# ThorsteinnJonsson/SLAM_framework

Hardware: AMD Instinct MI355X
Metric: stereo frames/sec ORB extract+match @1241x376, 2000 kp/frame (higher is better)
Workload: dtype u8; 1 GPU; configs[1]: synthetic 1241x376 stereo stream, 2000 kp/frame, extract L+R + stereo match + frame-to-frame match; batch=256, streams=1, batches_in_flight=2, nfeatures=2000, nlevels=8, parallelism=frame-sharded x1

## Files before the change

### slam_framework_amd/csrc/orb_kernels.hip

```cpp
#include <hip/hip_runtime.h>
#include <stdint.h>

#include <type_traits>
#include <utility>
#include <cstdlib>

#include "device_math.h"
#include "timing.h"
#include "orb_geometry.h"
#include "orb_kernels.h"

namespace slamgpu {

__constant__ __attribute__((aligned(16))) int8_t c_pattern[1024] = {
#include "orb_pattern.inc"
};

__device__ __forceinline__ const uint8_t* level_ptr(const ImageBatch& b, const OrbGeom* g,
                                                    int img, int level, int* pitch) {
  if (level == 0) {
    *pitch = b.in_pitch;
    return batch_image(b, img);
  }
  *pitch = g->lv[level].pitch;
// ... 992 lines not shown
      const int U = block_scan_array<kThr>(S.b, m, S.wsum);
      const int E = block_scan_array<kThr>(S.c, m, S.wsum);
      const int newm = T + U;
      const int seq0 = S.seq_next;
      const bool ovf = newm > min(2 * L.node_cap, kOctCap) || E > kOctCap;
      if (!ovf) {
        for (int j = tid; j < m; j += kThr) {
          const OctNode nd = Lc[j];
          if (nd.n > 1) {
            int gpos = S.a[j], epos = S.c[j];
            for (int q = 0; q < 4; q++) {
              OctNode ch = child[4 * j + q];
              if (ch.n == 0) continue;
              ch.seq = seq0 + gpos;
              const int pos = T - 1 - gpos;
              Ln[pos] = ch;
              if (ch.n > 1) S.sortk[epos++] = (uint64_t)pos;
              gpos++;
            }
          } else {
            Ln[T + S.b[j]] = nd;
          }
        }
      }
      __syncthreads();
      if (tid == 0) {
        if (ovf) {
          atomicOr(err, kErrNodeOverflow);
          S.finish = 1;
        } else {
          S.m = newm;
          S.seq_next = seq0 + T;
          S.nexp = E;
          if (newm >= N || newm == m) S.finish = 1;
          else if (newm + E * 3 > N) S.mode = 1;
        }
      }
      if (!ovf) cur ^= 1;
      __syncthreads();
      if (S.finish) break;
    } else {
      const int V = S.nexp;
      int P2 = 1;
      while (P2 < V) P2 <<= 1;
      for (int i = tid; i < P2; i += kThr) {
        uint64_t key = 0;
        if (i < V) {
          const int pos = (int)S.sortk[i];
          const OctNode& nd = Lc[pos];
          key = ((uint64_t)nd.n << 44) | ((uint64_t)(uint32_t)nd.seq << 12) | (uint64_t)pos;
        }
        S.sortk[i] = key;
      }
      __syncthreads();
      for (int k = 2; k <= P2; k <<= 1) {
        for (int jj = k >> 1; jj > 0; jj >>= 1) {
          for (int i = tid; i < P2; i += kThr) {
            const int ixj = i ^ jj;
            if (ixj > i) {
              const uint64_t x = S.sortk[i], y = S.sortk[ixj];
              const bool desc = (i & k) == 0;
              if (desc ? (x < y) : (x > y)) {
                S.sortk[i] = y;
                S.sortk[ixj] = x;
              }
            }
          }
          __syncthreads();
        }
      }
      for (int j = wid; j < V; j += (kThr / 64)) {
        const int pos = (int)(S.sortk[j] & 0xfff);
        const OctNode nd = Lc[pos];
        OctNode ch[4];
        divide_wave(nd, keys, ch, lane);
        if (lane == 0) {
          int t = 0, e = 0;
          for (int q = 0; q < 4; q++) {
            child[4 * j + q] = ch[q];
            t += ch[q].n > 0;
            e += ch[q].n > 1;
          }
          S.a[j] = t;
          S.c[j] = e;
          S.b[j] = t - 1;
        }
      }
      __syncthreads();
      for (int i = tid; i < V; i += kThr) S.b[i] = S.a[i] - 1;
      __syncthreads();
      block_scan_array<kThr>(S.b, V, S.wsum);
      if (tid == 0) S.total = V - 1;
      __syncthreads();
      for (int j = tid; j < V; j += kThr)
        if (m + S.b[j] + (S.a[j] - 1) >= N) atomicMin(&S.total, j);
      __syncthreads();
      const int J = S.total;
      const int nproc = J + 1;
      for (int i = tid; i < V; i += kThr)
        if (i >= nproc) {
          S.a[i] = 0;
          S.c[i] = 0;
        }
      __syncthreads();
      const int T = block_scan_array<kThr>(S.a, V, S.wsum);
      const int E = block_scan_array<kThr>(S.c, V, S.wsum);
      for (int i = tid; i < m; i += kThr) S.b[i] = 1;
      __syncthreads();
      for (int j = tid; j < nproc; j += kThr) S.b[(int)(S.sortk[j] & 0xfff)] = 0;
      __syncthreads();
      const int U = block_scan_array<kThr>(S.b, m, S.wsum);
      const int newm = T + U;
      const int seq0 = S.seq_next;
      const bool ovf = newm > min(2 * L.node_cap, kOctCap) || E > kOctCap;
      __shared__ uint8_t processed[kOctCap];
      for (int i = tid; i < m; i += kThr) processed[i] = 0;
      __syncthreads();
      for (int j = tid; j < nproc; j += kThr) processed[(int)(S.sortk[j] & 0xfff)] = 1;
      __syncthreads();
      __shared__ int vnext[kOctCap];
      if (!ovf) {
        for (int j = tid; j < nproc; j += kThr) {
          int gpos = S.a[j], epos = S.c[j];
          for (int q = 0; q < 4; q++) {
            OctNode ch = child[4 * j + q];
            if (ch.n == 0) continue;
            ch.seq = seq0 + gpos;
            const int pos = T - 1 - gpos;
            Ln[pos] = ch;
            if (ch.n > 1) vnext[epos++] = pos;
            gpos++;
          }
        }
        for (int i = tid; i < m; i += kThr)
          if (!processed[i]) Ln[T + S.b[i]] = Lc[i];
      }
      __syncthreads();
      for (int i = tid; i < E; i += kThr) S.sortk[i] = (uint64_t)vnext[i];
      __syncthreads();
      if (tid == 0) {
        if (ovf) {
          atomicOr(err, kErrNodeOverflow);
          S.finish = 1;
        } else {
          S.m = newm;
          S.seq_next = seq0 + T;
          S.nexp = E;
          if (newm >= N || newm == m) S.finish = 1;
        }
      }
      if (!ovf) cur ^= 1;
      __syncthreads();
      if (S.finish) break;
    }
  }
  const int m = S.m;
  const OctNode* Lf = lists[cur];
  const int mout = min(m, L.out_cap);
  for (int j = tid; j < mout; j += kThr) {
    const OctNode nd = Lf[j];
    const uint32_t* ks = keys[nd.buf] + nd.kbeg;
    uint32_t best = ks[0];
    for (int k = 1; k < nd.n; k++) {
      const uint32_t kk = ks[k];
      if (key_score(kk) > key_score(best)) best = kk;
    }
    outk[j] = best;
  }
  if (tid == 0) {
    if (m > L.out_cap) atomicOr(err, kErrNodeOverflow);
    *outc = mout;
  }
}

constexpr int kOctFbMaxGroups = 256;
__global__ __launch_bounds__(kOctThreads) void octree_kernel(
    const OrbGeom* __restrict__ g, int n_images, const uint32_t* __restrict__ cell_keys,
    const int* __restrict__ cell_count, uint32_t* __restrict__ key_scratch,
    OctNode* __restrict__ node_scratch, uint32_t* __restrict__ oct_keys,
    int* __restrict__ oct_count, uint32_t* __restrict__ err) {
  __shared__ OctShared S;
  __shared__ int s_todo[kOctThreads];
  __shared__ int s_wcnt[kOctWaves];
  const int tid = threadIdx.x, wid = tid >> 6, lane = tid & 63, nlev = g->nlevels;
  const int total = n_images * nlev;
  const int G = gridDim.x;
  for (int j0 = 0; (int)blockIdx.x + j0 * G < total; j0 += kOctThreads) {
    const int e = (int)blockIdx.x + (j0 + tid) * G;
    const bool redo = e < total && oct_count[e] == -1;
    const uint64_t m = __ballot(redo);
    if (lane == 0) s_wcnt[wid] = __popcll(m);
    __syncthreads();
    int off = 0, nt = 0;
    for (int w = 0; w < kOctWaves; w++) {
      if (w < wid) off += s_wcnt[w];
      nt += s_wcnt[w];
    }
    if (redo) s_todo[off + lanes_below(m)] = e;
    __syncthreads();
    for (int i = 0; i < nt; i++) {
      const int ei = s_todo[i];
      octree_global<kOctThreads>(S, ei % nlev, ei / nlev, g, cell_keys, cell_count, key_scratch,
                                 node_scratch, oct_keys, oct_count, err);
      __syncthreads();
    }
    __syncthreads();
  }
}

#ifndef OCT_PROF
#define OCT_PROF 0
#endif
#ifndef OCT_LANE_KEYS
#define OCT_LANE_KEYS 64
#endif
constexpr int kOctLaneKeys = OCT_LANE_KEYS;
constexpr int kOctDivRegs = 16;

struct OctNodeS {
  int16_t x0, x1, y0, y1;
  uint32_t kn;
};
static_assert(sizeof(OctNodeS) == 12, "compact node");
__device__ __forceinline__ int node_kbeg(const OctNodeS& d) { return (int)(d.kn & 0xffffu); }
__device__ __forceinline__ int node_n(const OctNodeS& d) { return (int)(d.kn >> 16); }

__device__ __forceinline__ OctNodeS readlane_node(const OctNodeS& nd, int l) {
  uint32_t w[3];
  __builtin_memcpy(w, &nd, sizeof(w));
#pragma unroll
  for (int i = 0; i < 3; i++) w[i] = (uint32_t)__builtin_amdgcn_readlane((int)w[i], l);
  OctNodeS o;
  __builtin_memcpy(&o, w, sizeof(w));
  return o;
}

__device__ __forceinline__ int quadrant(uint32_t k, int xm, int ym) {
  return (key_x(k) >= xm ? 1 : 0) + (key_y(k) >= ym ? 2 : 0);
}
__device__ __forceinline__ int node_xm(const OctNodeS& d) { return d.x0 + ((d.x1 - d.x0 + 1) >> 1); }
__device__ __forceinline__ int node_ym(const OctNodeS& d) { return d.y0 + ((d.y1 - d.y0 + 1) >> 1); }

__device__ __forceinline__ int wave_excl_scan(int v, int lane, int* total) {
  int x = v;
  x += __builtin_amdgcn_update_dpp(0, x, 0x111, 0xf, 0xf, false);
  x += __builtin_amdgcn_update_dpp(0, x, 0x112, 0xf, 0xf, false);
  x += __builtin_amdgcn_update_dpp(0, x, 0x114, 0xf, 0xf, false);
  x += __builtin_amdgcn_update_dpp(0, x, 0x118, 0xf, 0xf, false);
  x += __builtin_amdgcn_update_dpp(0, x, 0x142, 0xa, 0xf, false);
  x += __builtin_amdgcn_update_dpp(0, x, 0x143, 0xc, 0xf, false);
  *total = __builtin_amdgcn_readlane(x, 63);
  (void)lane;
  return x - v;
}

__device__ __forceinline__ int wave_scan_array(int16_t* a, int n, int lane) {
  int carry = 0;
  for (int c = 0; c < n; c += 64) {
    const int i = c + lane;
    const int v = i < n ? a[i] : 0;
    int tot;
    const int ex = wave_excl_scan(v, lane, &tot);
    if (i < n) a[i] = (int16_t)(carry + ex);
    carry += tot;
  }
  return carry;
}

__device__ __forceinline__ uint32_t lane_divide(const OctNodeS& nd, uint32_t* keys, bool part) {
  const int xm = node_xm(nd), ym = node_ym(nd), kb = node_kbeg(nd), n = node_n(nd);
  uint32_t kr[kOctLaneKeys];
  uint32_t c = 0;
#pragma unroll
  for (int r = 0; r < kOctLaneKeys; r++)
    if (r < n) {
      kr[r] = keys[kb + r];
      c += 1u << (8 * quadrant(kr[r], xm, ym));
    }
  if (part) {
    uint32_t run = (c << 8) + (c << 16) + (c << 24);
#pragma unroll
    for (int r = 0; r < kOctLaneKeys; r++)
      if (r < n) {
        const int q = quadrant(kr[r], xm, ym);
        keys[kb + ((run >> (8 * q)) & 255)] = kr[r];
        run += 1u << (8 * q);
      }
  }
  return c;
}

__device__ __forceinline__ void wave_count(const OctNodeS& nd, const uint32_t* keys, int lane,
                                           int cnt[4]) {
  const int xm = node_xm(nd), ym = node_ym(nd), kb = node_kbeg(nd), n = node_n(nd);
#pragma unroll
  for (int q = 0; q < 4; q++) cnt[q] = 0;
  for (int s0 = 0; s0 < n; s0 += 64) {
    const int q = s0 + lane < n ? quadrant(keys[kb + s0 + lane], xm, ym) : -1;
#pragma unroll
    for (int qq = 0; qq < 4; qq++) cnt[qq] += __popcll(__ballot(q == qq));
  }
}

__device__ void wave_partition(const OctNodeS& nd, uint32_t* keys, uint32_t* gscratch, int lane,
                               int cnt[4]) {
  const int xm = node_xm(nd), ym = node_ym(nd), kb = node_kbeg(nd), n = node_n(nd);
  if (n <= 64 * kOctDivRegs) {
    const int R = (n + 63) >> 6;
    uint32_t kr[kOctDivRegs];
    int qr[kOctDivRegs];
#pragma unroll
    for (int r = 0; r < kOctDivRegs; r++) {
      qr[r] = -1;
      if (r < R && 64 * r + lane < n) {
        kr[r] = keys[kb + 64 * r + lane];
        qr[r] = quadrant(kr[r], xm, ym);
      }
    }
#pragma unroll
    for (int q = 0; q < 4; q++) cnt[q] = 0;
#pragma unroll
    for (int r = 0; r < kOctDivRegs; r++)
      if (r < R) {
#pragma unroll
        for (int q = 0; q < 4; q++) cnt[q] += __popcll(__ballot(qr[r] == q));
      }
    int run[4] = {0, cnt[0], cnt[0] + cnt[1], cnt[0] + cnt[1] + cnt[2]};
#pragma unroll
    for (int r = 0; r < kOctDivRegs; r++)
      if (r < R) {
#pragma unroll
        for (int q = 0; q < 4; q++) {
          const uint64_t m = __ballot(qr[r] == q);
          if (qr[r] == q) keys[kb + run[q] + lanes_below(m)] = kr[r];
          run[q] += __popcll(m);
        }
      }
  } else {
    wave_count(nd, keys, lane, cnt);
    int run[4] = {0, cnt[0], cnt[0] + cnt[1], cnt[0] + cnt[1] + cnt[2]};
    for (int i = lane; i < n; i += 64) gscratch[kb + i] = keys[kb + i];
    __builtin_amdgcn_fence(__ATOMIC_SEQ_CST, "agent");
    for (int s0 = 0; s0 < n; s0 += 64) {
      const int i = s0 + lane;
      uint32_t k = 0;
      int q = -1;
      if (i < n) {
        k = gscratch[kb + i];
        q = quadrant(k, xm, ym);
      }
#pragma unroll
      for (int qq = 0; qq < 4; qq++) {
        const uint64_t m = __ballot(q == qq);
        if (q == qq) keys[kb + run[qq] + lanes_below(m)] = k;
        run[qq] += __popcll(m);
      }
    }
  }
}

__global__ __launch_bounds__(64 * kMaxLevels) void octree_img_kernel(
    const OrbGeom* __restrict__ g, const uint32_t* __restrict__ cell_keys,
    const int* __restrict__ cell_count, uint32_t* __restrict__ key_scratch,
    uint32_t* __restrict__ oct_keys, int* __restrict__ oct_count, uint32_t* __restrict__ err) {
  extern __shared__ __attribute__((aligned(16))) uint8_t s_oct[];
  __shared__ int s_K[kMaxLevels];
  const int img = blockIdx.x, lane = threadIdx.x & 63, level = wave_id();
  const int nlev = g->nlevels;
  const bool active = level < nlev;
  const LevelGeom& L = g->lv[active ? level : 0];
  const int ncell = L.ncols * L.nrows;
  const int64_t cbase = (int64_t)img * g->cells_per_image + L.cell_base;
#if OCT_PROF
  uint64_t op_t = clock64(), op_acc[8] = {0, 0, 0, 0, 0, 0, 0, 0};
  int op_np = 0, op_V = 0;
  uint32_t op_pass[8][6] = {};
  auto optick = [&](int i) {
    const uint64_t t = clock64();
    op_acc[i] += t - op_t;
    if (i >= 2 && i <= 5 && op_np >= 1 && op_np <= 8) op_pass[op_np - 1][i] += (uint32_t)(t - op_t);
    op_t = t;
  };
#else
  auto optick = [](int) {};
#endif
  int K = 0;
  if (active) {
    for (int c = lane; c < ncell; c += 64) K += cell_count[cbase + c];
    K = wave_sum(K);
    if (lane == 0) s_K[level] = K;
  }
  __syncthreads();
  if (!active) return;
  optick(0);
  int* const outc = oct_count + img * nlev + level;
  uint32_t* const outk = oct_keys + (int64_t)img * g->out_per_image + L.out_base;
  const int nIni = L.n_ini;
  int koff = 0;
  bool fits = true;
  for (int l = 0; l <= level; l++) {
    const bool f = koff + s_K[l] <= g->oct_kcap;
    if (l == level) fits = f;
    else if (f) koff += s_K[l];
  }
  if (!fits || nIni > 16) {
    if (lane == 0) *outc = -1;
    return;
  }
  if (K == 0) {
    if (lane == 0) *outc = 0;
    return;
  }
  uint32_t* const keys = reinterpret_cast<uint32_t*>(s_oct) + koff;
  uint32_t* const gscratch = key_scratch + img * g->keys_per_image + L.key_base;
  const int NC = L.oct_nc;
  OctNodeS* const lists = reinterpret_cast<OctNodeS*>(s_oct + L.oct_list_off);
  uint32_t* const sortk = reinterpret_cast<uint32_t*>(s_oct + L.oct_work_off);
  int16_t* const pt = reinterpret_cast<int16_t*>(sortk + NC);
  int16_t* const pe = pt + NC;
  int16_t* const pu = pe + NC;
  int16_t* const vnext = pu + NC;
  uint8_t* const processed = reinterpret_cast<uint8_t*>(vnext + NC);

  const float hX = L.hx;
  constexpr int kGatherChunks = 8, kGatherRegs = 48;
  constexpr int kMaxGroups = 64 * kGatherChunks / kCellGroup;
  static_assert(kMaxGroups >= 2 && (kMaxGroups & (kMaxGroups - 1)) == 0,
                "the gather's binary search halves its step from kMaxGroups / 2 down to 1");
  static_assert(kMaxGroups <= 64 * kGatherChunks,
                "gp[] (one int per key group) must fit the ncell + 1 <= NC sort keys it borrows");
  int bcnt = 0;
  if (ncell <= 64 * kGatherChunks && K <= 64 * kGatherRegs && ncell + 1 <= NC) {
    int* const gp = reinterpret_cast<int*>(sortk);
    int ccnt[kGatherChunks];
#pragma unroll
    for (int ch = 0; ch < kGatherChunks; ch++) {
      const int c = 64 * ch + lane;
      ccnt[ch] = c < ncell ? cell_count[cbase + c] : 0;
    }
    int carry = 0;
#pragma unroll
    for (int ch = 0; ch < kGatherChunks; ch++) {
      if (64 * ch < ncell) {
        int ctot;
        const int cex = wave_excl_scan(ccnt[ch], lane, &ctot);
        const int c = 64 * ch + lane;
        if (c < ncell && (c & (kCellGroup - 1)) == 0) gp[c / kCellGroup] = carry + cex;
        carry += ctot;
      }
    }
    __builtin_amdgcn_fence(__ATOMIC_SEQ_CST, "wavefront");
    __builtin_amdgcn_wave_barrier();
    const int R = (K + 63) >> 6;
    const int ng = (ncell + kCellGroup - 1) / kCellGroup;
    uint32_t kr[kGatherRegs];
    int br[kGatherRegs];
#pragma unroll
    for (int r = 0; r < kGatherRegs; r++) br[r] = 0;
#pragma unroll
    for (int step = kMaxGroups / 2; step >= 1; step >>= 1) {
#pragma unroll
      for (int r = 0; r < kGatherRegs; r++) {
        if (r < R) {
          const int cand = br[r] + step;
          if (cand < ng && gp[cand] <= 64 * r + lane) br[r] = cand;
        }
      }
    }
#pragma unroll
    for (int r = 0; r < kGatherRegs; r++) {
      const int s = 64 * r + lane;
      if (r < R && s < K)
        kr[r] = cell_keys[(cbase + kCellGroup * br[r]) * g->cell_cap + (s - gp[br[r]])];
      br[r] = -1;
    }
#pragma unroll
    for (int r = 0; r < kGatherRegs; r++) {
      if (r < R && 64 * r + lane < K) {
        br[r] = (int)((float)key_x(kr[r]) / hX);
        if (br[r] >= nIni) br[r] = -1;
      }
    }
#pragma unroll
    for (int r = 0; r < kGatherRegs; r++)
      if (r < R)
        for (int bb = 0; bb < nIni; bb++) {
          const int pc = __popcll(__ballot(br[r] == bb));
          if (lane == bb) bcnt += pc;
        }
    int tot;
    int brun = wave_excl_scan(lane < nIni ? bcnt : 0, lane, &tot);
#pragma unroll
    for (int r = 0; r < kGatherRegs; r++)
      if (r < R)
        for (int bb = 0; bb < nIni; bb++) {
          const uint64_t mm = __ballot(br[r] == bb);
          const int at = __builtin_amdgcn_readlane(brun, bb);
          if (br[r] == bb) keys[at + lanes_below(mm)] = kr[r];
          if (lane == bb) brun += __popcll(mm);
        }
  } else {
    for (int sweep = 0; sweep < 2; sweep++) {
      int brun = 0;
      if (sweep == 1) {
        int tot;
        brun = wave_excl_scan(lane < nIni ? bcnt : 0, lane, &tot);
      }
      for (int c0 = 0; c0 < ncell; c0 += 64) {
        const int cnt = c0 + lane < ncell ? cell_count[cbase + c0 + lane] : 0;
        int ctot;
        const int cex = wave_excl_scan(cnt, lane, &ctot);
        for (int r0 = 0; r0 < ctot; r0 += 64) {
          const int r = r0 + lane;
          int lo = 0;
#pragma unroll
          for (int step = 32; step >= 1; step >>= 1) {
            const int cand = lo + step;
            const int pv = __shfl(cex, cand & 63, 64);
            if (cand < 64 && pv <= r) lo = cand;
          }
          const int gs = lo & ~(kCellGroup - 1);
          const int base = __shfl(cex, gs, 64);
          int b = -1;
          uint32_t k = 0;
          if (r < ctot) {
            k = cell_keys[(cbase + c0 + gs) * g->cell_cap + (r - base)];
            b = (int)((float)key_x(k) / hX);
            if (b >= nIni) b = -1;
          }
          for (int bb = 0; bb < nIni; bb++) {
            const uint64_t m = __ballot(b == bb);
            if (sweep == 1) {
              const int at = __builtin_amdgcn_readlane(brun, bb);
              if (b == bb) keys[at + lanes_below(m)] = k;
              if (lane == bb) brun += __popcll(m);
            } else if (lane == bb) {
              bcnt += __popcll(m);
            }
          }
        }
      }
    }
  }
  int m = 0;
  {
    int tot;
    const int bbase = wave_excl_scan(lane < nIni ? bcnt : 0, lane, &tot);
    const bool has = lane < nIni && bcnt > 0;
    const uint64_t hm = __ballot(has);
    if (has) {
      OctNodeS nd;
      nd.x0 = (int16_t)(int)(hX * (float)lane);
      nd.x1 = (int16_t)(int)(hX * (float)(lane + 1));
      nd.y0 = 0;
      nd.y1 = (int16_t)(L.max_by - kMinBorder);
      nd.kn = (uint32_t)bbase | (uint32_t)bcnt << 16;
      lists[lanes_below(hm)] = nd;
    }
    m = __popcll(hm);
  }
  optick(1);
  const int N = L.budget;
  int cur = 0, nexp = 0;
  bool outer = true;
  while (true) {
    const OctNodeS* Lc = lists + cur * NC;
    OctNodeS* Ln = lists + (cur ^ 1) * NC;
    const int V = outer ? m : nexp;
#if OCT_PROF
    op_np++;
    op_V += V;
    if (op_np <= 8) op_pass[op_np - 1][0] = V;
#endif
    if (!outer) {
      int P2 = 64;
      while (P2 < V) P2 <<= 1;
      for (int i = lane; i < P2; i += 64) {
        uint32_t key = 0;
        if (i < V) {
          const int pos = (int)sortk[i];
          key = (uint32_t)node_n(Lc[pos]) << 12 | (uint32_t)(4095 - pos);
        }
        sortk[i] = key;
      }
      for (int k = 2; k <= P2; k <<= 1)
        for (int jj = k >> 1; jj > 0; jj >>= 1) {
          __builtin_amdgcn_fence(__ATOMIC_SEQ_CST, "wavefront");
          __builtin_amdgcn_wave_barrier();
          for (int i = lane; i < P2; i += 64) {
            const int ixj = i ^ jj;
            if (ixj > i) {
              const uint32_t x = sortk[i], y = sortk[ixj];
              const bool desc = (i & k) == 0;
              if (desc ? (x < y) : (x > y)) {
                sortk[i] = y;
                sortk[ixj] = x;
              }
            }
          }
        }
      __builtin_amdgcn_fence(__ATOMIC_SEQ_CST, "wavefront");
      __builtin_amdgcn_wave_barrier();
    }
    optick(2);
    auto nidx = [&](int j) { return outer ? j : 4095 - (int)(sortk[j] & 0xfffu); };
    for (int j0 = 0; j0 < V; j0 += 64) {
      const int j = j0 + lane;
      const bool valid = j < V;
      OctNodeS nd{};
      if (valid) nd = Lc[nidx(j)];
      const int n = node_n(nd);
      int t = 0, e = 0;
      if (valid && n > 1 && n <= kOctLaneKeys) {
        const uint32_t c = lane_divide(nd, keys, false);
#pragma unroll
        for (int q = 0; q < 4; q++) {
          const int cq = (c >> (8 * q)) & 255;
          t += cq > 0;
          e += cq > 1;
        }
      }
      uint64_t bigm = __ballot(valid && n > kOctLaneKeys);
#if OCT_PROF
      if (op_np <= 8) op_pass[op_np - 1][1] += __popcll(bigm);
#endif
      while (bigm) {
        const int bl = __builtin_ctzll(bigm);
        bigm &= bigm - 1;
        const OctNodeS nb = readlane_node(nd, bl);
        int cnt[4];
        wave_count(nb, keys, lane, cnt);
        if (lane == bl) {
#pragma unroll
          for (int q = 0; q < 4; q++) {
            t += cnt[q] > 0;
            e += cnt[q] > 1;
          }
        }
      }
      if (valid) {
        pt[j] = (int16_t)t;
        pe[j] = (int16_t)e;
        pu[j] = (int16_t)(outer ? (n == 1) : t - 1);
      }
    }
    optick(3);
    int nproc = V;
    if (!outer) {
      int carry = 0;
      nproc = V;
      for (int j0 = 0; j0 < V; j0 += 64) {
        const int j = j0 + lane;
        const int v = j < V ? pu[j] : 0;
        int tot;
        const int incl = carry + wave_excl_scan(v, lane, &tot) + v;
        const uint64_t hit = __ballot(j < V && m + incl >= N);
        if (hit) {
          nproc = j0 + __builtin_ctzll(hit) + 1;
          break;
        }
        carry += tot;
      }
      for (int i = lane; i < m; i += 64) processed[i] = 0;
      __builtin_amdgcn_fence(__ATOMIC_SEQ_CST, "wavefront");
      __builtin_amdgcn_wave_barrier();
      for (int j = lane; j < nproc; j += 64) processed[nidx(j)] = 1;
      __builtin_amdgcn_fence(__ATOMIC_SEQ_CST, "wavefront");
      __builtin_amdgcn_wave_barrier();
      for (int i = lane; i < m; i += 64) pu[i] = (int16_t)(processed[i] ? 0 : 1);
    }
    __builtin_amdgcn_fence(__ATOMIC_SEQ_CST, "wavefront");
    __builtin_amdgcn_wave_barrier();
    const int T = wave_scan_array(pt, nproc, lane);
    const int E = wave_scan_array(pe, nproc, lane);
    const int U = wave_scan_array(pu, m, lane);
    const int newm = T + U;
    if (newm > NC || E > NC) {
      if (lane == 0) atomicOr(err, kErrNodeOverflow);
      break;
    }
    __builtin_amdgcn_fence(__ATOMIC_SEQ_CST, "wavefront");
    __builtin_amdgcn_wave_barrier();
    optick(4);
    auto place = [&](int j, const OctNodeS& nd, uint32_t c4) {
      int gpos = pt[j], epos = pe[j];
      const int xm = node_xm(nd), ym = node_ym(nd);
      const int16_t xs[3] = {nd.x0, (int16_t)xm, nd.x1};
      const int16_t ys[3] = {nd.y0, (int16_t)ym, nd.y1};
      int start = node_kbeg(nd);
#pragma unroll
      for (int q = 0; q < 4; q++) {
        const int cq = (int)((c4 >> (8 * q)) & 255u);
        if (cq > 0) {
          OctNodeS ch;
          ch.x0 = xs[q & 1];
          ch.x1 = xs[(q & 1) + 1];
          ch.y0 = ys[q >> 1];
          ch.y1 = ys[(q >> 1) + 1];
          ch.kn = (uint32_t)start | (uint32_t)cq << 16;
          const int pos = T - 1 - gpos;
          Ln[pos] = ch;
          if (cq > 1) vnext[epos++] = (int16_t)pos;
          gpos++;
        }
        start += cq;
      }
    };
    for (int j0 = 0; j0 < nproc; j0 += 64) {
      const int j = j0 + lane;
      const bool valid = j < nproc;
      OctNodeS nd{};
      if (valid) nd = Lc[nidx(j)];
      const int n = node_n(nd);
      if (valid && n > 1 && n <= kOctLaneKeys) place(j, nd, lane_divide(nd, keys, true));
      uint64_t bigm = __ballot(valid && n > kOctLaneKeys);
      while (bigm) {
        const int bl = __builtin_ctzll(bigm);
        bigm &= bigm - 1;
        const OctNodeS nb = readlane_node(nd, bl);
        const int gpos0 = pt[j0 + bl], epos0 = pe[j0 + bl];
        int cnt[4];
        wave_partition(nb, keys, gscratch, lane, cnt);
        if (lane == 0) {
          int gpos = gpos0, epos = epos0;
          const int xm = node_xm(nb), ym = node_ym(nb);
          const int16_t xs[3] = {nb.x0, (int16_t)xm, nb.x1};
          const int16_t ys[3] = {nb.y0, (int16_t)ym, nb.y1};
          int start = node_kbeg(nb);
          for (int q = 0; q < 4; q++) {
            if (cnt[q] > 0) {
              OctNodeS ch;
              ch.x0 = xs[q & 1];
              ch.x1 = xs[(q & 1) + 1];
              ch.y0 = ys[q >> 1];
              ch.y1 = ys[(q >> 1) + 1];
              ch.kn = (uint32_t)start | (uint32_t)cnt[q] << 16;
              const int pos = T - 1 - gpos;
              Ln[pos] = ch;
              if (cnt[q] > 1) vnext[epos++] = (int16_t)pos;
              gpos++;
            }
            start += cnt[q];
          }
        }
      }
    }
    for (int i = lane; i < m; i += 64) {
      const OctNodeS nd = Lc[i];
      if (outer ? node_n(nd) == 1 : !processed[i]) Ln[T + pu[i]] = nd;
    }
    __builtin_amdgcn_fence(__ATOMIC_SEQ_CST, "wavefront");
    __builtin_amdgcn_wave_barrier();
    for (int i = lane; i < E; i += 64) sortk[i] = (uint32_t)vnext[i];
    optick(5);
    const int mprev = m;
    m = newm;
    nexp = E;
    cur ^= 1;
    if (newm >= N || newm == mprev) break;
    if (outer && newm + E * 3 > N) outer = false;
  }
  __builtin_amdgcn_fence(__ATOMIC_SEQ_CST, "wavefront");
  __builtin_amdgcn_wave_barrier();
  const OctNodeS* Lf = lists + cur * NC;
  const int mout = min(m, L.out_cap);
  for (int j = lane; j < mout; j += 64) {
    const OctNodeS nd = Lf[j];
    const int kb = node_kbeg(nd), n = node_n(nd);
    uint32_t best = keys[kb];
    for (int k = 1; k < n; k++) {
      const uint32_t kk = keys[kb + k];
      if (key_score(kk) > key_score(best)) best = kk;
    }
    outk[j] = best;
  }
  if (lane == 0) {
    if (m > L.out_cap) atomicOr(err, kErrNodeOverflow);
    *outc = mout;
  }
#if OCT_PROF
  optick(6);
  if (lane == 0 && img < 2)
    printf("[octprof] img %d level %d K %d passes %d V %d | cyc: count %llu gather %llu sort %llu "
           "count %llu scan %llu place %llu retain %llu\n", img, level, K, op_np, op_V,
           (unsigned long long)op_acc[0], (unsigned long long)op_acc[1],
           (unsigned long long)op_acc[2], (unsigned long long)op_acc[3],
           (unsigned long long)op_acc[4], (unsigned long long)op_acc[5],
           (unsigned long long)op_acc[6]);
  if (lane == 0 && img == 0 && level == 0)
    for (int i = 0; i < op_np && i < 8; i++)
      printf("[octpass] pass %d V %u big %u sort %u count %u scan %u place %u\n", i,
             op_pass[i][0], op_pass[i][1], op_pass[i][2], op_pass[i][3], op_pass[i][4], op_pass[i][5]);
#endif
}

constexpr int kOctLvlWaves = 8, kOctLvlThreads = 64 * kOctLvlWaves;
constexpr int kOctKpt = 16;
#ifndef OCT_LVL_MAX_IMAGES
#define OCT_LVL_MAX_IMAGES 16
#endif
constexpr int kOctLvlMaxImages = OCT_LVL_MAX_IMAGES;

__device__ __forceinline__ int lvl_block_sum(int v, int* red) {
  v = wave_sum(v);
  if ((threadIdx.x & 63) == 0) red[wave_id()] = v;
  __syncthreads();
  int t = 0;
#pragma unroll
  for (int k = 0; k < kOctLvlWaves; k++) t += red[k];
  __syncthreads();
  return t;
}

__device__ void lvl_block_scan(int* a, int n, int* red) {
  const int lane = threadIdx.x & 63, w = wave_id();
  int carry = 0;
  for (int c = 0; c < n; c += kOctLvlThreads) {
    const int i = c + (int)threadIdx.x;
    const int v = i < n ? a[i] : 0;
    int wt;
    const int ex = wave_excl_scan(v, lane, &wt);
    if (lane == 0) red[w] = wt;
    __syncthreads();
    int pre = 0, tot = 0;
#pragma unroll
    for (int k = 0; k < kOctLvlWaves; k++) {
      pre += k < w ? red[k] : 0;
      tot += red[k];
    }
    if (i < n) a[i] = carry + pre + ex;
    carry += tot;
    __syncthreads();
  }
}

__global__ __launch_bounds__(kOctLvlThreads) void octree_lvl_kernel(
    const OrbGeom* __restrict__ g, const uint32_t* __restrict__ cell_keys,
    const int* __restrict__ cell_count, uint32_t* __restrict__ key_scratch,
    OctNode* __restrict__ node_scratch, uint32_t* __restrict__ oct_keys,
    int* __restrict__ oct_count, uint32_t* __restrict__ err) {
  extern __shared__ __attribute__((aligned(16))) uint8_t s_lvl[];
  __shared__ int s_red[kOctLvlWaves];
  __shared__ int s_bc[kOctLvlWaves][16];
  __shared__ int s_brun[16];
  __shared__ int s_bcnt[16];
  __shared__ int s_u[4];
  __shared__ int s_scan[kOctLvlWaves][2];
  const int level = blockIdx.x, img = blockIdx.y;
  const int tid = threadIdx.x, lane = tid & 63, w = wave_id();
  const int nlev = g->nlevels;
  const LevelGeom& L = g->lv[level];
  const int ncell = L.ncols * L.nrows;
  const int64_t cbase = (int64_t)img * g->cells_per_image + L.cell_base;
  int* const outc = oct_count + img * nlev + level;
  auto otick = [](int) {};
  uint32_t* const outk = oct_keys + (int64_t)img * g->out_per_image + L.out_base;
  int K = 0;
  for (int c = tid; c < ncell; c += kOctLvlThreads) K += cell_count[cbase + c];
  K = lvl_block_sum(K, s_red);
  const int nIni = L.n_ini;
  const int NC = L.oct_nc;
  if (K > g->oct2_kcap || K > kOctKpt * kOctLvlThreads || nIni > 16 ||
      ncell + 1 > g->oct2_ccap || NC > g->oct2_nc) {
    if (tid == 0) *outc = -1;
    __syncthreads();
    octree_global<kOctLvlThreads>(*reinterpret_cast<OctShared*>(s_lvl), level, img, g, cell_keys,
                                  cell_count, key_scratch, node_scratch, oct_keys, oct_count, err);
    return;
  }
  if (K == 0) {
    if (tid == 0) *outc = 0;
    return;
  }
  uint32_t* const keys = reinterpret_cast<uint32_t*>(s_lvl);
  uint32_t* const tmp = reinterpret_cast<uint32_t*>(s_lvl + g->oct2_tmp_off);
  int* const cpre = reinterpret_cast<int*>(s_lvl + g->oct2_cpre_off);
  OctNodeS* const lists = reinterpret_cast<OctNodeS*>(s_lvl + g->oct2_list_off);
  uint32_t* const sortk = reinterpret_cast<uint32_t*>(s_lvl + g->oct2_work_off);
  int16_t* const pt = reinterpret_cast<int16_t*>(sortk + NC);
  int16_t* const pe = pt + NC;
  int16_t* const pu = pe + NC;
  int16_t* const vnext = pu + NC;
  uint8_t* const processed = reinterpret_cast<uint8_t*>(vnext + NC);
  uint8_t* const cand = processed + NC;
  uint2* const nst = reinterpret_cast<uint2*>(
      (reinterpret_cast<uintptr_t>(cand + NC) + 15) & ~static_cast<uintptr_t>(15));
  uint2* const nen = nst + NC;
  int16_t* const cb = reinterpret_cast<int16_t*>(nen + NC);

  for (int c = tid; c < ncell; c += kOctLvlThreads) cpre[c] = cell_count[cbase + c];
  if (tid < 16) s_bcnt[tid] = 0;
  __syncthreads();
  lvl_block_scan(cpre, ncell, s_red);
  const float hX = L.hx;
  auto bucket = [&](uint32_t k) {
    const int b = (int)((float)key_x(k) / hX);
    return b >= nIni ? -1 : b;
  };
  constexpr int kGatherUnroll = 4;
  for (int s0 = 0; s0 < K; s0 += kGatherUnroll * kOctLvlThreads) {
    uint32_t kr[kGatherUnroll];
    int sr[kGatherUnroll];
#pragma unroll
    for (int r = 0; r < kGatherUnroll; r++) {
      const int s = s0 + r * kOctLvlThreads + tid;
      sr[r] = s;
      if (s < K) {
        int lo = 0, hi = ncell;
        while (hi - lo > 1) {
          const int mid = (lo + hi) >> 1;
          if (cpre[mid] <= s) lo = mid;
          else hi = mid;
        }
        const int gs = lo & ~(kCellGroup - 1);
        kr[r] = cell_keys[(cbase + gs) * g->cell_cap + (s - cpre[gs])];
      }
    }
#pragma unroll
    for (int r = 0; r < kGatherUnroll; r++)
      if (sr[r] < K) {
        tmp[sr[r]] = kr[r];
        const int b = bucket(kr[r]);
        if (b >= 0) atomicAdd(&s_bcnt[b], 1);
      }
  }
  __syncthreads();
  if (w == 0) {
    int tot;
    const int bb = wave_excl_scan(lane < nIni ? s_bcnt[lane] : 0, lane, &tot);
    if (lane < 16) s_brun[lane] = bb;
  }
  __syncthreads();
  for (int s0 = 0; s0 < K; s0 += kOctLvlThreads) {
    const int s = s0 + tid;
    uint32_t k = 0;
    int b = -1;
    if (s < K) {
      k = tmp[s];
      b = bucket(k);
    }
    int rank = 0;
    for (int bb = 0; bb < nIni; bb++) {
      const uint64_t m = __ballot(b == bb);
      if (b == bb) rank = lanes_below(m);
      if (lane == bb) s_bc[w][bb] = __popcll(m);
    }
    __syncthreads();
    if (b >= 0) {
      int pos = s_brun[b] + rank;
      for (int k2 = 0; k2 < w; k2++) pos += s_bc[k2][b];
      keys[pos] = k;
    }
    __syncthreads();
    if (tid < nIni) {
      int add = 0;
#pragma unroll
      for (int k2 = 0; k2 < kOctLvlWaves; k2++) add += s_bc[k2][tid];
      s_brun[tid] += add;
    }
    __syncthreads();
  }
  if (w == 0) {
    const int bcnt = lane < nIni ? s_bcnt[lane] : 0;
    int tot;
    const int bbase = wave_excl_scan(bcnt, lane, &tot);
    const bool has = lane < nIni && bcnt > 0;
    const uint64_t hm = __ballot(has);
    if (has) {
      OctNodeS nd;
      nd.x0 = (int16_t)(int)(hX * (float)lane);
      nd.x1 = (int16_t)(int)(hX * (float)(lane + 1));
      nd.y0 = 0;
      nd.y1 = (int16_t)(L.max_by - kMinBorder);
      nd.kn = (uint32_t)bbase | (uint32_t)bcnt << 16;
      lists[lanes_below(hm)] = nd;
    }
    if (lane == 0) s_u[0] = __popcll(hm);
  }
  __syncthreads();
  int m = s_u[0];
  __syncthreads();

  otick(0);
  const int N = L.budget;
  int cur = 0, nexp = 0;
  bool outer = true;
  int Kn = 0;
  for (int i = 0; i < m; i++) Kn += node_n(lists[i]);
  const int kpt = (Kn + kOctLvlThreads - 1) / kOctLvlThreads;
  const int kb0 = tid * kpt;
  uint32_t kr[kOctKpt];
  int nd[kOctKpt];
  uint32_t plo[kOctKpt], phi[kOctKpt];
  uint64_t qbits = 0;
#pragma unroll
  for (int i = 0; i < kOctKpt; i++) {
    nd[i] = 0;
    if (i < kpt && kb0 + i < Kn) {
      const int k = kb0 + i;
      kr[i] = keys[k];
      int c = 0;
      for (int q = 1; q < m; q++) c += node_kbeg(lists[q]) <= k;
      nd[i] = c;
    }
  }
  while (true) {
    const OctNodeS* Lc = lists + cur * NC;
    OctNodeS* Ln = lists + (cur ^ 1) * NC;
    const int V = outer ? m : nexp;
    if (!outer) {
      int P2 = 64;
      while (P2 < V) P2 <<= 1;
      for (int i = tid; i < P2; i += kOctLvlThreads) {
        uint32_t key = 0;
        if (i < V) {
          const int pos = (int)sortk[i];
          key = (uint32_t)node_n(Lc[pos]) << 12 | (uint32_t)(4095 - pos);
        }
        sortk[i] = key;
      }
      for (int i = tid; i < m; i += kOctLvlThreads) cand[i] = 0;
      __syncthreads();
      for (int i = tid; i < V; i += kOctLvlThreads) cand[4095 - (int)(sortk[i] & 0xfffu)] = 1;
      __syncthreads();
      if (V <= 2 * kOctLvlThreads) {
        uint32_t mine[2];
        int rk[2] = {0, 0};
#pragma unroll
        for (int r = 0; r < 2; r++) {
          const int i = tid + r * kOctLvlThreads;
          mine[r] = i < V ? sortk[i] : 0u;
        }
        const uint4* s4 = reinterpret_cast<const uint4*>(sortk);
        for (int j4 = 0; j4 < P2 / 4; j4++) {
          const uint4 o = s4[j4];
#pragma unroll
          for (int r = 0; r < 2; r++)
            rk[r] += (int)(o.x > mine[r]) + (int)(o.y > mine[r]) + (int)(o.z > mine[r]) +
                     (int)(o.w > mine[r]);
        }
        __syncthreads();
#pragma unroll
        for (int r = 0; r < 2; r++)
          if (tid + r * kOctLvlThreads < V) sortk[rk[r]] = mine[r];
        __syncthreads();
      } else {
        for (int k = 2; k <= P2; k <<= 1)
          for (int jj = k >> 1; jj > 0; jj >>= 1) {
            for (int i = tid; i < P2; i += kOctLvlThreads) {
              const int ixj = i ^ jj;
              if (ixj > i) {
                const uint32_t x = sortk[i], y = sortk[ixj];
                const bool desc = (i & k) == 0;
                if (desc ? (x < y) : (x > y)) {
                  sortk[i] = y;
                  sortk[ixj] = x;
                }
              }
            }
            __syncthreads();
          }
      }
    }
    otick(1);
    auto nidx = [&](int j) { return outer ? j : 4095 - (int)(sortk[j] & 0xfffu); };
    auto is_cand = [&](int i, const OctNodeS& nn) { return outer ? node_n(nn) > 1 : cand[i] != 0; };
    uint32_t slo = 0, shi = 0;
    qbits = 0;
#pragma unroll
    for (int i = 0; i < kOctKpt; i++) {
      if (i < kpt) {
        uint32_t olo = 0, ohi = 0;
        if (kb0 + i < Kn) {
          const OctNodeS nn = Lc[nd[i]];
          if (is_cand(nd[i], nn)) {
            const uint32_t q = (uint32_t)quadrant(kr[i], node_xm(nn), node_ym(nn));
            qbits |= (uint64_t)q << (2 * i);
            const uint32_t oh = 1u << (16 * (q & 1));
            olo = q < 2 ? oh : 0u;
            ohi = q < 2 ? 0u : oh;
          }
        }
        plo[i] = slo;
        phi[i] = shi;
        slo += olo;
        shi += ohi;
      }
    }
    {
      int tl, th;
      const int el = wave_excl_scan((int)slo, lane, &tl);
// ... 847 lines not shown
```

Measured before the change: 111,800 stereo frames/s.

## Pre-bin octree keys into two quadtree levels during gather and sort in registers

The octree gather now computes each key's initial-column bin plus two levels of quadrant subdivision up front, then places keys with an LDS radix-style counting sort using packed byte histograms. This lets the first one or two octree subdivision passes skip per-node key partitioning and use binary-search counts instead. The small-V bitonic node sort moves from LDS into registers with shuffles, and lane_divide results are cached in the outer pass. It also adds a waves-per-EU occupancy hint and force-inlines wave_partition. The cost is much more code, extra register pressure and fallback gating conditions.

Result: no change. 112,300 stereo frames/s (median of 6 runs) (+0.4%).

```diff
diff --git a/slam_framework_amd/csrc/orb_kernels.hip b/slam_framework_amd/csrc/orb_kernels.hip
--- a/slam_framework_amd/csrc/orb_kernels.hip
+++ b/slam_framework_amd/csrc/orb_kernels.hip
@@ -1318,8 +1318,8 @@
   }
 }
 
-__device__ void wave_partition(const OctNodeS& nd, uint32_t* keys, uint32_t* gscratch, int lane,
-                               int cnt[4]) {
+__device__ __forceinline__ void wave_partition(const OctNodeS& nd, uint32_t* keys,
+                                               uint32_t* gscratch, int lane, int cnt[4]) {
   const int xm = node_xm(nd), ym = node_ym(nd), kb = node_kbeg(nd), n = node_n(nd);
   if (n <= 64 * kOctDivRegs) {
     const int R = (n + 63) >> 6;
@@ -1375,7 +1375,110 @@
   }
 }
 
-__global__ __launch_bounds__(64 * kMaxLevels) void octree_img_kernel(
+template <int N, class F>
+__device__ __forceinline__ void for_regs(int R, F&& f) {
+#pragma unroll
+  for (int r8 = 0; r8 < N; r8 += 8)
+    if (r8 < R) {
+#pragma unroll
+      for (int r = r8; r < (r8 + 8 < N ? r8 + 8 : N); r++)
+        if (r < R) f(r);
+    }
+}
+
+__device__ __forceinline__ void wave_lds_sync() {
+  __builtin_amdgcn_fence(__ATOMIC_SEQ_CST, "wavefront");
+  __builtin_amdgcn_wave_barrier();
+}
+
+template <int C>
+__device__ __forceinline__ void regs_sort_vprev(uint32_t* sortk, const OctNodeS* Lc, int V, int P2,
+                                                int lane) {
+  uint32_t sv[C];
+#pragma unroll
+  for (int c = 0; c < C; c++) {
+    sv[c] = 0;
+    const int i = 64 * c + lane;
+    if (i < V) {
+      const int pos = (int)sortk[i];
+      sv[c] = (uint32_t)node_n(Lc[pos]) << 12 | (uint32_t)(4095 - pos);
+    }
+  }
+#pragma unroll
+  for (int lk = 1; lk <= 9; lk++) {
+    const int k = 1 << lk;
+    if (k > 64 * C || k > P2) break;
+#pragma unroll
+    for (int lj = lk - 1; lj >= 0; lj--) {
+      const int jj = 1 << lj;
+      if (jj >= 64) {
+        const int cj = jj >> 6;
+#pragma unroll
+        for (int c = 0; c < C; c++)
+          if ((c & cj) == 0 && (c | cj) < C) {
+            const uint32_t x = sv[c], y = sv[c | cj];
+            const bool desc = ((64 * c) & k) == 0;
+            sv[c] = desc ? max(x, y) : min(x, y);
+            sv[c | cj] = desc ? min(x, y) : max(x, y);
+          }
+      } else {
+        uint32_t y[C];
+#pragma unroll
+        for (int c = 0; c < C; c++) y[c] = (uint32_t)__shfl_xor((int)sv[c], jj, 64);
+        const bool up = (lane & jj) != 0;
+#pragma unroll
+        for (int c = 0; c < C; c++) {
+          const bool desc = ((64 * c + lane) & k) == 0;
+          sv[c] = desc != up ? max(sv[c], y[c]) : min(sv[c], y[c]);
+        }
+      }
+    }
+  }
+  wave_lds_sync();
+#pragma unroll
+  for (int c = 0; c < C; c++)
+    if (64 * c < P2) sortk[64 * c + lane] = sv[c];
+}
+
+__device__ __forceinline__ int oct_key_bin(uint32_t k, float hX, int nIni, int ym, int ym_lo,
+                                           int ym_hi) {
+  const int x = key_x(k), y = key_y(k);
+  const int b = (int)((float)x / hX);
+  if (b >= nIni) return -1;
+  const int x0 = (int16_t)(int)(hX * (float)b), x1 = (int16_t)(int)(hX * (float)(b + 1));
+  const int xm = x0 + ((x1 - x0 + 1) >> 1);
+  const int qx = x >= xm ? 1 : 0, qy = y >= ym ? 1 : 0;
+  const int lo = qx ? xm : x0, hi = qx ? x1 : xm;
+  const int xm2 = lo + ((hi - lo + 1) >> 1);
+  const int qx2 = x >= xm2 ? 1 : 0, qy2 = y >= (qy ? ym_hi : ym_lo) ? 1 : 0;
+  return b * 16 + (qx + 2 * qy) * 4 + (qx2 + 2 * qy2);
+}
+
+__device__ __forceinline__ void sorted_node_counts(const OctNodeS& nd, const uint32_t* keys,
+                                                   int cnt[4]) {
+  const int xm = node_xm(nd), ym = node_ym(nd), kb = node_kbeg(nd), n = node_n(nd);
+  int lt[3];
+#pragma unroll
+  for (int q = 1; q < 4; q++) {
+    int lo = 0, hi = n;
+    while (lo < hi) {
+      const int mid = (lo + hi) >> 1;
+      if (quadrant(keys[kb + mid], xm, ym) < q) lo = mid + 1;
+      else hi = mid;
+    }
+    lt[q - 1] = lo;
+  }
+  cnt[0] = lt[0];
+  cnt[1] = lt[1] - lt[0];
+  cnt[2] = lt[2] - lt[1];
+  cnt[3] = n - lt[2];
+}
+
+#ifndef OCT_IMG_WAVES_PER_EU
+#define OCT_IMG_WAVES_PER_EU 4
+#endif
+__global__ __launch_bounds__(64 * kMaxLevels)
+__attribute__((amdgpu_waves_per_eu(OCT_IMG_WAVES_PER_EU))) void octree_img_kernel(
     const OrbGeom* __restrict__ g, const uint32_t* __restrict__ cell_keys,
     const int* __restrict__ cell_count, uint32_t* __restrict__ key_scratch,
     uint32_t* __restrict__ oct_keys, int* __restrict__ oct_count, uint32_t* __restrict__ err) {
@@ -1397,8 +1500,16 @@
     if (i >= 2 && i <= 5 && op_np >= 1 && op_np <= 8) op_pass[op_np - 1][i] += (uint32_t)(t - op_t);
     op_t = t;
   };
+  uint64_t og_acc[6] = {0, 0, 0, 0, 0, 0};
+  auto ogtick = [&](int i) {
+    const uint64_t t = clock64();
+    og_acc[i] += t - op_t;
+    op_acc[1] += t - op_t;
+    op_t = t;
+  };
 #else
   auto optick = [](int) {};
+  auto ogtick = [](int) {};
 #endif
   int K = 0;
   if (active) {
@@ -1446,7 +1557,9 @@
   static_assert(kMaxGroups <= 64 * kGatherChunks,
                 "gp[] (one int per key group) must fit the ncell + 1 <= NC sort keys it borrows");
   int bcnt = 0;
-  if (ncell <= 64 * kGatherChunks && K <= 64 * kGatherRegs && ncell + 1 <= NC) {
+  int pre = 0;
+  if (ncell <= 64 * kGatherChunks && K <= 64 * kGatherRegs && ncell + 1 <= NC && nIni <= 15 &&
+      64 * ((max(4, nIni) + 3) & ~3) <= 12 * NC) {
     int* const gp = reinterpret_cast<int*>(sortk);
     int ccnt[kGatherChunks];
 #pragma unroll
@@ -1465,56 +1578,144 @@
         carry += ctot;
       }
     }
-    __builtin_amdgcn_fence(__ATOMIC_SEQ_CST, "wavefront");
-    __builtin_amdgcn_wave_barrier();
-    const int R = (K + 63) >> 6;
+    wave_lds_sync();
+    const int Rs = (K + 63) >> 6;
     const int ng = (ncell + kCellGroup - 1) / kCellGroup;
-    uint32_t kr[kGatherRegs];
-    int br[kGatherRegs];
-#pragma unroll
-    for (int r = 0; r < kGatherRegs; r++) br[r] = 0;
+    constexpr int kRunRegs = kGatherRegs + 1;
+    uint32_t kr[kRunRegs];
+    uint32_t bp[(kRunRegs + 3) / 4];
+#pragma unroll
+    for (int r = 0; r < kGatherRegs; r++) kr[r] = 0;
 #pragma unroll
     for (int step = kMaxGroups / 2; step >= 1; step >>= 1) {
-#pragma unroll
-      for (int r = 0; r < kGatherRegs; r++) {
-        if (r < R) {
-          const int cand = br[r] + step;
-          if (cand < ng && gp[cand] <= 64 * r + lane) br[r] = cand;
-        }
-      }
-    }
-#pragma unroll
-    for (int r = 0; r < kGatherRegs; r++) {
-      const int s = 64 * r + lane;
-      if (r < R && s < K)
-        kr[r] = cell_keys[(cbase + kCellGroup * br[r]) * g->cell_cap + (s - gp[br[r]])];
-      br[r] = -1;
-    }
-#pragma unroll
-    for (int r = 0; r < kGatherRegs; r++) {
-      if (r < R && 64 * r + lane < K) {
-        br[r] = (int)((float)key_x(kr[r]) / hX);
-        if (br[r] >= nIni) br[r] = -1;
-      }
-    }
-#pragma unroll
-    for (int r = 0; r < kGatherRegs; r++)
-      if (r < R)
-        for (int bb = 0; bb < nIni; bb++) {
-          const int pc = __popcll(__ballot(br[r] == bb));
-          if (lane == bb) bcnt += pc;
-        }
-    int tot;
-    int brun = wave_excl_scan(lane < nIni ? bcnt : 0, lane, &tot);
-#pragma unroll
-    for (int r = 0; r < kGatherRegs; r++)
-      if (r < R)
-        for (int bb = 0; bb < nIni; bb++) {
-          const uint64_t mm = __ballot(br[r] == bb);
-          const int at = __builtin_amdgcn_readlane(brun, bb);
-          if (br[r] == bb) keys[at + lanes_below(mm)] = kr[r];
-          if (lane == bb) brun += __popcll(mm);
-        }
+      for_regs<kGatherRegs>(Rs, [&](int r) {
+        const int cand = (int)kr[r] + step;
+        if (cand < ng && gp[cand] <= 64 * r + lane) kr[r] = (uint32_t)cand;
+      });
+    }
+    for_regs<kGatherRegs>(Rs, [&](int r) {
+      const int s = 64 * r + lane, gr = (int)kr[r];
+      if (s < K) kr[r] = cell_keys[(cbase + kCellGroup * gr) * g->cell_cap + (s - gp[gr])];
+    });
+    for_regs<kGatherRegs>(Rs, [&](int r) {
+      if (64 * r + lane < K) keys[64 * r + lane] = kr[r];
+    });
+    ogtick(0);
+    const int R = Rs | 1, s0 = lane * R;
+    const int H = L.max_by - kMinBorder;
+    const int ym = (H + 1) >> 1, ym_lo = (ym + 1) >> 1, ym_hi = ym + ((H - ym + 1) >> 1);
+    uint8_t* const tbl = reinterpret_cast<uint8_t*>(lists);
+    uint32_t* const cnt = reinterpret_cast<uint32_t*>(tbl);
+    uint32_t* const o32 = reinterpret_cast<uint32_t*>(tbl);
+    for (int i = lane; i < 16 * nIni; i += 64) cnt[i] = 0;
+    const bool wide = 64 * nIni <= 3 * NC, wide2 = nIni <= 4 && 256 * nIni <= 3 * NC;
+    int sh = -1, Kcur = K;
+    while (true) {
+      wave_lds_sync();
+      for_regs<kRunRegs>(R, [&](int r) {
+        int bin = -1;
+        if (s0 + r < Kcur) {
+          kr[r] = keys[s0 + r];
+          bin = oct_key_bin(kr[r], hX, nIni, ym, ym_lo, ym_hi);
+          if (sh < 0 && bin >= 0)
+            __hip_atomic_fetch_add(&cnt[bin], 1u, __ATOMIC_RELAXED, __HIP_MEMORY_SCOPE_WAVEFRONT);
+        }
+        const int at = 8 * (r & 3);
+        bp[r >> 2] = (bp[r >> 2] & ~(0xffu << at)) | ((uint32_t)bin & 0xffu) << at;
+      });
+      wave_lds_sync();
+      ogtick(1);
+      if (sh < 0) {
+        int c2[4] = {0, 0, 0, 0}, c1 = 0;
+        if (lane < 4 * nIni) {
+#pragma unroll
+          for (int q = 0; q < 4; q++) {
+            c2[q] = (int)cnt[4 * lane + q];
+            c1 += c2[q];
+          }
+        }
+        int nb = c1 + __shfl_xor(c1, 1, 64);
+        nb += __shfl_xor(nb, 2, 64);
+        const bool first = (lane & 3) == 0;
+        const int N0 = L.budget;
+        const int m0 = __popcll(__ballot(first && nb > 0));
+        const int T0 = __popcll(__ballot(nb > 1 && c1 > 0)), E0 = __popcll(__ballot(c1 > 1));
+        const int newm0 = T0 + __popcll(__ballot(first && nb == 1));
+        if (T0 > 0 && newm0 <= NC && E0 <= NC) {
+          pre = 1;
+          if (newm0 < N0 && newm0 != m0 && newm0 + 3 * E0 <= N0) {
+            int t1 = 0, e1 = 0;
+#pragma unroll
+            for (int q = 0; q < 4; q++) {
+              t1 += c1 > 1 && c2[q] > 0;
+              e1 += c2[q] > 1;
+            }
+            const int newm1 = wave_sum(t1) + __popcll(__ballot(c1 == 1));
+            if (newm1 <= NC && wave_sum(e1) <= NC) pre = 2;
+          }
+        }
+        bcnt = __shfl(nb, (4 * lane) & 63, 64);
+        if (lane >= nIni) bcnt = 0;
+        Kcur = wave_sum(bcnt);
+        sh = 4 - 2 * pre;
+        wave_lds_sync();
+        ogtick(2);
+      }
+      const bool last = sh == 4 || (sh == 2 && wide) || wide2;
+      const int nbin = last ? nIni << (4 - sh) : 4, mask = last ? 0xfff : 3;
+      const int wpl = (nbin + 3) >> 2;
+      uint32_t* const h32 = o32 + 64 * wpl;
+      for (int i = lane; i < 64 * wpl; i += 64) h32[i] = 0;
+      wave_lds_sync();
+      for_regs<kRunRegs>(R, [&](int r) {
+        const int bin = (int)((bp[r >> 2] >> (8 * (r & 3))) & 0xffu);
+        if (bin != 0xff)
+          __hip_atomic_fetch_add(&h32[((bin >> sh) & mask) * 16 + (lane >> 2)],
+                                 1u << (8 * (lane & 3)), __ATOMIC_RELAXED,
+                                 __HIP_MEMORY_SCOPE_WAVEFRONT);
+      });
+      wave_lds_sync();
+      ogtick(3);
+      {
+        uint32_t hw[16];
+        int sum = 0;
+#pragma unroll
+        for (int i = 0; i < 16; i++) {
+          hw[i] = 0;
+          if (i < wpl) {
+            hw[i] = h32[lane * wpl + i];
+            sum += (int)__builtin_amdgcn_sad_u8(hw[i], 0u, 0u);
+          }
+        }
+        wave_lds_sync();
+        int tot;
+        uint32_t run = (uint32_t)wave_excl_scan(sum, lane, &tot);
+#pragma unroll
+        for (int i = 0; i < 16; i++)
+          if (i < wpl) {
+            const uint32_t w = hw[i], a = run + (w & 255u), b = a + ((w >> 8) & 255u),
+                           c = b + ((w >> 16) & 255u);
+            o32[2 * (lane * wpl + i)] = run | a << 16;
+            o32[2 * (lane * wpl + i) + 1] = b | c << 16;
+            run = c + (w >> 24);
+          }
+      }
+      wave_lds_sync();
+      ogtick(4);
+      for_regs<kRunRegs>(R, [&](int r) {
+        const int bin = (int)((bp[r >> 2] >> (8 * (r & 3))) & 0xffu);
+        if (bin != 0xff) {
+          const int idx = ((bin >> sh) & mask) * 64 + lane, hs = 16 * (idx & 1);
+          const uint32_t old = __hip_atomic_fetch_add(&o32[idx >> 1], 1u << hs, __ATOMIC_RELAXED,
+                                                      __HIP_MEMORY_SCOPE_WAVEFRONT);
+          keys[(old >> hs) & 0xffffu] = kr[r];
+        }
+      });
+      ogtick(5);
+      if (last) break;
+      sh += 2;
+    }
+    wave_lds_sync();
   } else {
     for (int sweep = 0; sweep < 2; sweep++) {
       int brun = 0;
@@ -1588,33 +1789,99 @@
     op_V += V;
     if (op_np <= 8) op_pass[op_np - 1][0] = V;
 #endif
+    if (pre > 0) {
+      pre--;
+      optick(2);
+      OctNodeS nd{};
+      if (lane < V) nd = Lc[lane];
+      const int n = node_n(nd);
+      int cq[4] = {0, 0, 0, 0}, t = 0, e = 0;
+      if (n > 1) {
+        sorted_node_counts(nd, keys, cq);
+#pragma unroll
+        for (int q = 0; q < 4; q++) {
+          t += cq[q] > 0;
+          e += cq[q] > 1;
+        }
+      }
+      optick(3);
+      int T, E, U;
+      int gpos = wave_excl_scan(t, lane, &T);
+      int epos = wave_excl_scan(e, lane, &E);
+      const int upos = wave_excl_scan(n == 1 ? 1 : 0, lane, &U);
+      const int newm = T + U;
+      if (newm > NC || E > NC) {
+        if (lane == 0) atomicOr(err, kErrNodeOverflow);
+        break;
+      }
+      optick(4);
+      if (n > 1) {
+        const int xm = node_xm(nd), ym = node_ym(nd);
+        const int16_t xs[3] = {nd.x0, (int16_t)xm, nd.x1};
+        const int16_t ys[3] = {nd.y0, (int16_t)ym, nd.y1};
+        int start = node_kbeg(nd);
+#pragma unroll
+        for (int q = 0; q < 4; q++) {
+          if (cq[q] > 0) {
+            OctNodeS ch;
+            ch.x0 = xs[q & 1];
+            ch.x1 = xs[(q & 1) + 1];
+            ch.y0 = ys[q >> 1];
+            ch.y1 = ys[(q >> 1) + 1];
+            ch.kn = (uint32_t)start | (uint32_t)cq[q] << 16;
+            const int pos = T - 1 - gpos;
+            Ln[pos] = ch;
+            if (cq[q] > 1) sortk[epos++] = (uint32_t)pos;
+            gpos++;
+          }
+          start += cq[q];
+        }
+      } else if (n == 1) {
+        Ln[T + upos] = nd;
+      }
+      wave_lds_sync();
+      optick(5);
+      const int mprev = m;
+      m = newm;
+      nexp = E;
+      cur ^= 1;
+      if (newm >= N || newm == mprev) break;
+      if (newm + E * 3 > N) outer = false;
+      continue;
+    }
     if (!outer) {
       int P2 = 64;
       while (P2 < V) P2 <<= 1;
-      for (int i = lane; i < P2; i += 64) {
-        uint32_t key = 0;
-        if (i < V) {
-          const int pos = (int)sortk[i];
-          key = (uint32_t)node_n(Lc[pos]) << 12 | (uint32_t)(4095 - pos);
-        }
-        sortk[i] = key;
-      }
-      for (int k = 2; k <= P2; k <<= 1)
-        for (int jj = k >> 1; jj > 0; jj >>= 1) {
-          __builtin_amdgcn_fence(__ATOMIC_SEQ_CST, "wavefront");
-          __builtin_amdgcn_wave_barrier();
-          for (int i = lane; i < P2; i += 64) {
-            const int ixj = i ^ jj;
-            if (ixj > i) {
-              const uint32_t x = sortk[i], y = sortk[ixj];
-              const bool desc = (i & k) == 0;
-              if (desc ? (x < y) : (x > y)) {
-                sortk[i] = y;
-                sortk[ixj] = x;
+      if (P2 <= 256) {
+        regs_sort_vprev<4>(sortk, Lc, V, P2, lane);
+      } else if (P2 <= 512) {
+        regs_sort_vprev<8>(sortk, Lc, V, P2, lane);
+      } else {
+        for (int i = lane; i < P2; i += 64) {
+          uint32_t key = 0;
+          if (i < V) {
+            const int pos = (int)sortk[i];
+            key = (uint32_t)node_n(Lc[pos]) << 12 | (uint32_t)(4095 - pos);
+          }
+          sortk[i] = key;
+        }
+        for (int k = 2; k <= P2; k <<= 1)
+          for (int jj = k >> 1; jj > 0; jj >>= 1) {
+            __builtin_amdgcn_fence(__ATOMIC_SEQ_CST, "wavefront");
+            __builtin_amdgcn_wave_barrier();
+            for (int i = lane; i < P2; i += 64) {
+              const int ixj = i ^ jj;
+              if (ixj > i) {
+                const uint32_t x = sortk[i], y = sortk[ixj];
+                const bool desc = (i & k) == 0;
+                if (desc ? (x < y) : (x > y)) {
+                  sortk[i] = y;
+                  sortk[ixj] = x;
+                }
               }
             }
           }
-        }
+      }
       __builtin_amdgcn_fence(__ATOMIC_SEQ_CST, "wavefront");
       __builtin_amdgcn_wave_barrier();
     }
@@ -1628,7 +1895,8 @@
       const int n = node_n(nd);
       int t = 0, e = 0;
       if (valid && n > 1 && n <= kOctLaneKeys) {
-        const uint32_t c = lane_divide(nd, keys, false);
+        const uint32_t c = lane_divide(nd, keys, outer);
+        if (outer) sortk[j] = c;
 #pragma unroll
         for (int q = 0; q < 4; q++) {
           const int cq = (c >> (8 * q)) & 255;
@@ -1728,7 +1996,8 @@
       OctNodeS nd{};
       if (valid) nd = Lc[nidx(j)];
       const int n = node_n(nd);
-      if (valid && n > 1 && n <= kOctLaneKeys) place(j, nd, lane_divide(nd, keys, true));
+      if (valid && n > 1 && n <= kOctLaneKeys)
+        place(j, nd, outer ? sortk[j] : lane_divide(nd, keys, true));
       uint64_t bigm = __ballot(valid && n > kOctLaneKeys);
       while (bigm) {
         const int bl = __builtin_ctzll(bigm);
@@ -1803,6 +2072,11 @@
            (unsigned long long)op_acc[2], (unsigned long long)op_acc[3],
            (unsigned long long)op_acc[4], (unsigned long long)op_acc[5],
            (unsigned long long)op_acc[6]);
+  if (lane == 0 && img == 0)
+    printf("[octgath] level %d K %d | cyc: load %llu bins %llu gate %llu hist %llu scan %llu place %llu\n",
+           level, K, (unsigned long long)og_acc[0], (unsigned long long)og_acc[1],
+           (unsigned long long)og_acc[2], (unsigned long long)og_acc[3],
+           (unsigned long long)og_acc[4], (unsigned long long)og_acc[5]);
   if (lane == 0 && img == 0 && level == 0)
     for (int i = 0; i < op_np && i < 8; i++)
       printf("[octpass] pass %d V %u big %u sort %u count %u scan %u place %u\n", i,
```
